# brown-palm/goal-force

Measured on AMD Instinct MI355X. Metric: frames_per_sec (81-frame video / (50-step denoise loop + VAE decode), Wan2.2-I2V-A14B 832x480x81f), higher is better.
Workload: dtype bf16

## Files before the change

goal_force_amd/csrc/gf_cross_fold.hip:

```cpp
#include "gf_common.h"

namespace {

constexpr int CF_HD = 128;
constexpr int CF_MAXK = 64;
constexpr int CF_THREADS = 256;
constexpr int CF_QB = 128;

__device__ __forceinline__ void cf_mfma32(f32x16& acc, const bf16x8& a, const bf16x8& b) {
    acc = __builtin_amdgcn_mfma_f32_32x32x16_bf16(a, b, acc, 0, 0, 0);
}

__global__ __launch_bounds__(CF_THREADS) void cross_probs_kernel(const u16* __restrict__ q, const u16* __restrict__ k, u16* __restrict__ pout,
                                                                 int q_len, int n_keys, int n_pad, int heads, long q_stride, long k_stride,
                                                                 long p_stride, float c, float last_key_bias) {
    __shared__ __attribute__((aligned(16))) char lds[CF_MAXK * 256];
    const int tid = threadIdx.x;
    const int lane = tid & 63, wave = tid >> 6;
    const int r = lane & 31, h = lane >> 5;
    const int head = blockIdx.y;
    const int q0 = blockIdx.x * CF_QB + wave * 32;
    const int halves = n_keys > 32 ? 2 : 1;

#pragma unroll
// ... 2 lines not shown
        const int row = idx >> 4, ch = idx & 15;
        u16x8 v8 = {0, 0, 0, 0, 0, 0, 0, 0};
        if (row < n_keys) v8 = *reinterpret_cast<const u16x8*>(k + (long)row * k_stride + head * CF_HD + ch * 8);
        const int sk = ((row & 3) << 2) | ((row >> 2) & 3);
        *(u16x8*)(lds + row * 256 + ((ch ^ sk) << 4)) = v8;
    }

    bf16x8 qf[8];
    {
        const int qr = min(q0 + r, q_len - 1);
        const u16* qp = q + (long)qr * q_stride + head * CF_HD + 8 * h;
#pragma unroll
        for (int kd = 0; kd < 8; ++kd) qf[kd] = *reinterpret_cast<const bf16x8*>(qp + 16 * kd);
    }
    __syncthreads();

    f32x16 sc[2];
#pragma unroll
    for (int e = 0; e < 16; ++e) {
        sc[0][e] = 0.f;
        sc[1][e] = 0.f;
    }
    const int sK = ((r & 3) << 2) | ((r >> 2) & 3);
#pragma unroll
    for (int kd = 0; kd < 8; ++kd) {
        const int off = 256 * r + 16 * ((2 * kd + h) ^ sK);
        cf_mfma32(sc[0], *(const bf16x8*)(lds + off), qf[kd]);
        if (halves == 2) cf_mfma32(sc[1], *(const bf16x8*)(lds + off + 32 * 256), qf[kd]);
    }

#pragma unroll
    for (int e = 0; e < 16; ++e) {
        const int key = 4 * h + (e & 3) + 8 * (e >> 2);
        if (key >= n_keys) sc[0][e] = -INFINITY;
        if (key + 32 >= n_keys) sc[1][e] = -INFINITY;
        if (key == n_keys - 1) sc[0][e] += last_key_bias;
        if (key + 32 == n_keys - 1) sc[1][e] += last_key_bias;
    }
    float mx = sc[0][0];
#pragma unroll
    for (int e = 1; e < 16; ++e) mx = fmaxf(mx, sc[0][e]);
#pragma unroll
    for (int e = 0; e < 16; ++e) mx = fmaxf(mx, sc[1][e]);
    mx = fmaxf(mx, __shfl_xor(mx, 32));
    const float mc = mx * c;
    float rs = 0.f;
#pragma unroll
    for (int e = 0; e < 16; ++e) {
        sc[0][e] = __builtin_amdgcn_exp2f(__builtin_fmaf(sc[0][e], c, -mc));
        sc[1][e] = __builtin_amdgcn_exp2f(__builtin_fmaf(sc[1][e], c, -mc));
        rs += sc[0][e] + sc[1][e];
    }
    const float l_tot = rs + __shfl_xor(rs, 32);
    const float inv = 1.0f / l_tot;
    float pl = 0.f;
#pragma unroll
    for (int e = 0; e < 16; ++e) {
        const int key = 4 * h + (e & 3) + 8 * (e >> 2);
        if (key == n_keys - 1) pl = sc[0][e];
        if (key + 32 == n_keys - 1) pl = sc[1][e];
    }
    pl += __shfl_xor(pl, 32);
    const float wl = pl * inv;
    const float wl_lo = wl - bf2f(f2bf(wl));

    const int qrow = q0 + r;
    if (qrow < q_len) {
        u16* prow = pout + (long)qrow * p_stride + (long)head * n_pad;
#pragma unroll
        for (int half = 0; half < 2; ++half)
#pragma unroll
            for (int g = 0; g < 4; ++g) {
                const int key = 32 * half + 8 * g + 4 * h;
                if (key < n_pad) {
                    float w4[4];
#pragma unroll
                    for (int i = 0; i < 4; ++i) w4[i] = key + i == n_keys ? wl_lo : sc[half][4 * g + i] * inv;
                    u32x2 pk;
                    pk[0] = pack2bf(w4[0], w4[1]);
                    pk[1] = pack2bf(w4[2], w4[3]);
                    *reinterpret_cast<u32x2*>(prow + key) = pk;
                }
            }
    }
}

constexpr int CFT_ROWS = 64;
__global__ __launch_bounds__(CF_THREADS) void cross_fold_table_kernel(const u16* __restrict__ v, const u16* __restrict__ w, u16* __restrict__ u,
                                                                      int n_keys, int n_pad, int n_out, long v_stride, long w_stride,
                                                                      long u_stride) {
    __shared__ __attribute__((aligned(16))) u16 vs[CF_MAXK * CF_HD];
    const int tid = threadIdx.x;
    const int head = blockIdx.y;
    for (int idx = tid; idx < n_pad * 16; idx += CF_THREADS) {
        const int row = idx >> 4, ch = idx & 15;
        u16x8 v8 = {0, 0, 0, 0, 0, 0, 0, 0};
        if (row <= n_keys) v8 = *reinterpret_cast<const u16x8*>(v + (long)min(row, n_keys - 1) * v_stride + head * CF_HD + ch * 8);
        *reinterpret_cast<u16x8*>(vs + row * CF_HD + ch * 8) = v8;
    }
    __syncthreads();
    const int n = blockIdx.x * CFT_ROWS + (tid >> 2), jg = tid & 3;
    if (n >= n_out) return;
    const int nj = n_pad >> 2;
    float acc[CF_MAXK / 4];
#pragma unroll
    for (int i = 0; i < CF_MAXK / 4; ++i) acc[i] = 0.f;
    const u16* wr = w + (long)n * w_stride + head * CF_HD;
    for (int d0 = 0; d0 < CF_HD; d0 += 8) {
        const u16x8 w8 = *reinterpret_cast<const u16x8*>(wr + d0);
        float wf[8];
#pragma unroll
        for (int e = 0; e < 8; ++e) wf[e] = bf2f(w8[e]);
#pragma unroll
        for (int i = 0; i < CF_MAXK / 4; ++i) {
            if (i < nj) {
                const u16x8 v8 = *reinterpret_cast<const u16x8*>(vs + (jg + 4 * i) * CF_HD + d0);
#pragma unroll
                for (int e = 0; e < 8; ++e) acc[i] = __builtin_fmaf(bf2f(v8[e]), wf[e], acc[i]);
            }
        }
    }
    u16* ur = u + (long)n * u_stride + (long)head * n_pad;
#pragma unroll
    for (int i = 0; i < CF_MAXK / 4; ++i) {
        const int j = jg + 4 * i;
        if (i < nj) ur[j] = j <= n_keys ? f2bf(acc[i]) : (u16)0;
    }
}

}

extern "C" GF_API int gf_cross_probs(const void* q, const void* k, void* p, int64_t q_len, int64_t n_keys, int64_t n_pad, int64_t heads,
                                     int64_t head_dim, int64_t q_stride, int64_t k_stride, int64_t p_stride, float scale,
                                     float last_key_multiplicity, void* stream) {
    GF_CHECK_ARG(q && k && p, "gf_cross_probs: null pointer");
    if (head_dim != CF_HD) {
        gf_set_error("gf_cross_probs: head_dim=%ld unsupported (kernel is built for 128)", (long)head_dim);
        return GF_ERR_UNSUPPORTED;
    }
    GF_CHECK_ARG(q_len >= 0 && q_len < (1 << 30) && heads > 0 && heads < 65536, "gf_cross_probs: bad sizes q=%ld heads=%ld", (long)q_len,
                 (long)heads);
    GF_CHECK_ARG(n_keys >= 1 && n_pad % 16 == 0 && n_pad > n_keys && n_pad <= CF_MAXK,
                 "gf_cross_probs: 1 <= n_keys=%ld < n_pad=%ld <= 64, n_pad a multiple of 16", (long)n_keys, (long)n_pad);
    GF_CHECK_ARG(q_stride % 8 == 0 && k_stride % 8 == 0 && p_stride % 4 == 0 && q_stride >= heads * CF_HD && k_stride >= heads * CF_HD &&
                     p_stride >= heads * n_pad,
                 "gf_cross_probs: strides must cover the rows (q, k: multiples of 8; p: of 4, >= heads * n_pad)");
    GF_CHECK_ARG(gf_aligned16(q) && gf_aligned16(k) && ((uintptr_t)p & 7u) == 0, "gf_cross_probs: alignment (q, k 16 bytes, p 8 bytes)");
    GF_CHECK_ARG(scale > 0.f && last_key_multiplicity >= 1.0f, "gf_cross_probs: scale > 0, multiplicity >= 1");
    if (q_len == 0) return GF_OK;
    const float c = scale * 1.4426950408889634f;
    const float bias = last_key_multiplicity != 1.0f ? log2f(last_key_multiplicity) / c : 0.f;
    const dim3 grid((unsigned)((q_len + CF_QB - 1) / CF_QB), (unsigned)heads);
    hipLaunchKernelGGL(cross_probs_kernel, grid, dim3(CF_THREADS), 0, (hipStream_t)stream, (const u16*)q, (const u16*)k, (u16*)p,
                       (int)q_len, (int)n_keys, (int)n_pad, (int)heads, (long)q_stride, (long)k_stride, (long)p_stride, c, bias);
    GF_CHECK_LAUNCH("gf_cross_probs");
    return GF_OK;
}

extern "C" GF_API int gf_cross_fold_table(const void* v, const void* w_o, void* u, int64_t n_keys, int64_t n_pad, int64_t heads,
                                          int64_t head_dim, int64_t n_out, int64_t v_stride, int64_t w_stride, int64_t u_stride,
                                          void* stream) {
    GF_CHECK_ARG(v && w_o && u, "gf_cross_fold_table: null pointer");
    if (head_dim != CF_HD) {
        gf_set_error("gf_cross_fold_table: head_dim=%ld unsupported (kernel is built for 128)", (long)head_dim);
        return GF_ERR_UNSUPPORTED;
    }
    GF_CHECK_ARG(heads > 0 && heads < 65536 && n_out > 0 && n_out < (1 << 30), "gf_cross_fold_table: bad sizes heads=%ld N=%ld", (long)heads,
                 (long)n_out);
    GF_CHECK_ARG(n_keys >= 1 && n_pad % 16 == 0 && n_pad > n_keys && n_pad <= CF_MAXK,
                 "gf_cross_fold_table: 1 <= n_keys=%ld < n_pad=%ld <= 64, n_pad a multiple of 16", (long)n_keys, (long)n_pad);
    GF_CHECK_ARG(v_stride % 8 == 0 && w_stride % 8 == 0 && v_stride >= heads * CF_HD && w_stride >= heads * CF_HD && u_stride >= heads * n_pad,
                 "gf_cross_fold_table: strides must cover the rows (v, w_o: multiples of 8; u >= heads * n_pad)");
    GF_CHECK_ARG(gf_aligned16(v) && gf_aligned16(w_o) && ((uintptr_t)u & 1u) == 0, "gf_cross_fold_table: alignment");
    const dim3 grid((unsigned)((n_out + CFT_ROWS - 1) / CFT_ROWS), (unsigned)heads);
    hipLaunchKernelGGL(cross_fold_table_kernel, grid, dim3(CF_THREADS), 0, (hipStream_t)stream, (const u16*)v, (const u16*)w_o, (u16*)u,
                       (int)n_keys, (int)n_pad, (int)n_out, (long)v_stride, (long)w_stride, (long)u_stride);
    GF_CHECK_LAUNCH("gf_cross_fold_table");
    return GF_OK;
}
```

goal_force_amd/dit.py:

```python
from __future__ import annotations

import math
from typing import Optional, Tuple

import torch
import torch.nn as nn

from . import ops
from ._lib import GoalForceError


def precompute_freqs_cis(dim: int, end: int = 1024, theta: float = 10000.0):
    freqs = 1.0 / (theta ** (torch.arange(0, dim, 2)[: (dim // 2)].double() / dim))
    freqs = torch.outer(torch.arange(end), freqs)
    return torch.polar(torch.ones_like(freqs), freqs)


def precompute_freqs_cis_3d(dim: int, end: int = 1024, theta: float = 10000.0):
    return (precompute_freqs_cis(dim - 2 * (dim // 3), end, theta),
            precompute_freqs_cis(dim // 3, end, theta),
            precompute_freqs_cis(dim // 3, end, theta))


class RopeTable:
# ... 260 lines not shown
            q = linear(xin, self.q)
            ops.rmsnorm_rope(q, self.norm_q.weight, q_cos, q_sin, self.head_dim, self.norm_q.eps)
            hq = sp.heads_start(q, self.num_heads)
            return sp.attention_started(hq, hk, hv, self.num_heads, tuple(q.shape), scale=attn_scale, backend="sage" if sage else "flash")
        q, k = linear(xin, self.q), linear(xin, self.k)
        if keep is not None and keep.get("wide"):
            keep["qp"], keep["kp"] = q, k
            q, k = q.clone(), k.clone()
        ops.rmsnorm_rope(q, self.norm_q.weight, q_cos, q_sin, self.head_dim, self.norm_q.eps)
        ops.rmsnorm_rope(k, self.norm_k.weight, rope.cos, rope.sin, self.head_dim, self.norm_k.eps)
        if sp is None and keep is None and not fp8 and x2.is_cuda and self.v.weight.shape[0] >= 512 \
                and ops.vt32_ok(x2.shape[0], self.num_heads, self.head_dim):
            return attn(q, k, None, self.num_heads, vt=ops.linear_vt32(x2, self.v.weight, self.v.bias), scale=attn_scale)
        if sp is None and keep is None and fp8 and xin.is_cuda and self.v.weight.shape[0] >= 512 and self.v.weight.shape[1] % 128 == 0 \
                and ops.vt32_ok(xin.shape[0], self.num_heads, self.head_dim):
            if self.v._gf_w8_key != param_key(self.v.weight):
                self.v._gf_w8 = ops.cast_fp8(self.v.weight.detach().contiguous())
                self.v._gf_w8_key = param_key(self.v.weight)
            return attn(q, k, None, self.num_heads, vt=ops.linear_vt32_fp8(xin.x8, xin.scale, self.v._gf_w8, self.v.bias), scale=attn_scale)
        v = linear(xin, self.v)
        if sp is not None:
            return sp.attention(q, k, v, self.num_heads, scale=attn_scale, backend="sage" if sage else "flash")
        if keep is not None:
            keep["attn"], keep["lse"] = ops.flash_attn_lse(q, k, v, self.num_heads, scale=attn_scale)
            if keep.get("wide"):
                keep["v"] = v
            return keep["attn"]
        return attn(q, k, v, self.num_heads, scale=attn_scale)

    def forward(self, x, freqs):
        x2 = _tokens2d(x)
        a = self.attend(x2, _as_rope(freqs, x.device))
        return linear(a, self.o).view(x.shape)


class CrossAttention(nn.Module):

    def __init__(self, dim: int, num_heads: int, eps: float = 1e-6, has_image_input: bool = False):
        super().__init__()
        if has_image_input:
            raise NotImplementedError("has_image_input=True (CLIP image tokens) is outside the Goal-Force path")
        self.dim, self.num_heads, self.head_dim = dim, num_heads, dim // num_heads
        self.q, self.k, self.v, self.o = (nn.Linear(dim, dim) for _ in range(4))
        self.norm_q, self.norm_k = RMSNorm(dim, eps=eps), RMSNorm(dim, eps=eps)
        self.has_image_input = False

    def context_kv(self, ctx2: torch.Tensor, fold: bool = True, pad_n: Optional[int] = None):
        m = 1
        if fold and ctx2.is_cuda and ops._OPT["fold_pad_keys"]:
            n = pad_run(ctx2) if pad_n is None else pad_n
            if ctx2.shape[0] - n >= 2 and n + 1 < ops.VT_MIN_KV:
                m = ctx2.shape[0] - n
                ctx2 = ctx2[: n + 1]
        cin = QuantizedInput(ctx2) if getattr(self.k, "_gf_w8", None) is not None else ctx2
        k, v = linear(cin, self.k), linear(cin, self.v)
        ops.rmsnorm_rope(k, self.norm_k.weight, None, None, self.head_dim, self.norm_k.eps)
        return k, v, m

    def attend(self, x2, kv):
        q = linear(x2, self.q)
        ops.rmsnorm_rope(q, self.norm_q.weight, None, None, self.head_dim, self.norm_q.eps)
        return ops.flash_attn(q, kv[0], kv[1], self.num_heads, last_key_mult=kv[2] if len(kv) > 2 else 1)

    FOLD_K_MAX = 2560

    def fold_ok(self, kv) -> bool:
        if not ops._OPT["fold_cross_o"] or torch.is_grad_enabled() or len(kv) < 3 or kv[2] == 1 or self.head_dim != 128:
            return False
        if getattr(self.o, "_gf_w8", None) is not None:
            return False
        n = kv[0].shape[0]
        k = self.num_heads * self.fold_pad(n)
        return n <= ops.CROSS_FOLD_MAX_KEYS and k <= self.FOLD_K_MAX and k % 64 == 0

    @staticmethod
    def fold_pad(n_keys: int) -> int:
        return -(-(n_keys + 1) // 16) * 16

    def fold_table(self, kv):
        return ops.cross_fold_table(kv[1], self.o.weight, self.num_heads, self.fold_pad(kv[0].shape[0]))

    def attend_probs(self, x2, kv):
        q = linear(x2, self.q)
        ops.rmsnorm_rope(q, self.norm_q.weight, None, None, self.head_dim, self.norm_q.eps)
        return ops.cross_probs(q, kv[0], self.num_heads, self.fold_pad(kv[0].shape[0]), last_key_mult=kv[2])

    def forward(self, x: torch.Tensor, y: torch.Tensor):
        x2 = _tokens2d(x)
        a = self.attend(x2, self.context_kv(_tokens2d(y)))
        return linear(a, self.o).view(x.shape)


class GateModule(nn.Module):

    def forward(self, x, gate, residual):
        if x.shape != residual.shape:
            raise GoalForceError("GateModule: x and residual must have the same shape")
        d = x.shape[-1]
        g = gate.reshape(-1, d)
        if x.dim() == 3 and g.shape[0] == x.shape[0] and x.shape[0] > 1:
            return torch.stack([ops.gate_residual(x[b], g[b].contiguous(), residual[b]) for b in range(x.shape[0])])
        if g.shape[0] != 1:
            raise GoalForceError("GateModule: gate must be [B or 1, 1, D] (per-token gates are outside the Goal-Force path)")
        return ops.gate_residual(x, g[0].contiguous(), residual)


class DiTBlock(nn.Module):

    def __init__(self, has_image_input: bool, dim: int, num_heads: int, ffn_dim: int, eps: float = 1e-6):
        super().__init__()
        self.dim, self.num_heads, self.ffn_dim, self.eps = dim, num_heads, ffn_dim, eps
        self.self_attn = SelfAttention(dim, num_heads, eps)
        self.cross_attn = CrossAttention(dim, num_heads, eps, has_image_input=has_image_input)
        self.norm1 = nn.LayerNorm(dim, eps=eps, elementwise_affine=False)
        self.norm2 = nn.LayerNorm(dim, eps=eps, elementwise_affine=False)
        self.norm3 = nn.LayerNorm(dim, eps=eps)
        self.ffn = nn.Sequential(nn.Linear(dim, ffn_dim), nn.GELU(approximate="tanh"), nn.Linear(ffn_dim, dim))
        self.modulation = nn.Parameter(torch.randn(1, 6, dim) / dim ** 0.5)
        self.gate = GateModule()

    def forward(self, x, context, t_mod, freqs, context_kv=None, out=None, sp=None, keep=None, self_attn_memo=None,
                fold_pad_keys=True, pad_n=None, dense_attn=False):
        if t_mod.dim() == 4:
            raise NotImplementedError("per-token t_mod (seperated_timestep) is outside the Goal-Force path")
        x2 = _tokens2d(x)
        rope = _as_rope(freqs, x.device)
        mod = ops.modulation(self.modulation, t_mod.contiguous(), onep_mask=0b010010)
        fp8 = getattr(self.ffn[0], "_gf_w8", None) is not None
        if self_attn_memo is not None and "x" in self_attn_memo:
            x_new = self_attn_memo.pop("x")
            ev = self_attn_memo.pop("ev", None)
            if ev is not None:
                torch.cuda.current_stream(x_new.device).wait_event(ev)
                x_new.record_stream(torch.cuda.current_stream(x_new.device))
            if out is not None:
                x_new = out.copy_(x_new)
            h = None if fp8 else torch.empty_like(x2)
        else:
            if fp8:
                h = QuantizedInput.layernorm(x2, scale1p=mod[1], shift=mod[0], eps=self.eps)
            else:
                h = ops.layernorm_modulate(x2, scale1p=mod[1], shift=mod[0], eps=self.eps)
            a = self.self_attn.attend(h, rope, sp, keep, dense=dense_attn)
            x_new = out if out is not None else torch.empty_like(x2)
            linear(a, self.self_attn.o, epilogue=ops.EPI_BIAS_GATE_RESID, resid=x2, gate=mod[2], out=x_new)
            if keep is not None and keep.get("wide"):
                keep["x1"] = x_new.clone()
            if self_attn_memo is not None:
                self_attn_memo["x"] = x_new.clone()
                if x_new.is_cuda:
                    self_attn_memo["ev"] = torch.cuda.Event()
                    self_attn_memo["ev"].record(torch.cuda.current_stream(x_new.device))
        if fp8:
            h = QuantizedInput.layernorm(x_new, weight=self.norm3.weight, bias=self.norm3.bias, eps=self.eps)
        else:
            ops.layernorm_modulate(x_new, weight=self.norm3.weight, bias=self.norm3.bias, eps=self.eps, out=h)
        if context_kv is None:
            context_kv = self.cross_attn.context_kv(_tokens2d(context), fold=fold_pad_keys and keep is None, pad_n=pad_n)
        ca = self.cross_attn
        if keep is None and not fp8 and ca.fold_ok(context_kv):
            u = context_kv[3] if len(context_kv) > 3 else ca.fold_table(context_kv)
            ops.gemm(ca.attend_probs(h, context_kv), u, ca.o.bias, epilogue=ops.EPI_BIAS_RESID, resid=x_new, out=x_new)
        else:
            a = ca.attend(h, context_kv)
            linear(a, ca.o, epilogue=ops.EPI_BIAS_RESID, resid=x_new, out=x_new)
        if keep is not None and keep.get("wide"):
# ... 133 lines not shown
```

goal_force_amd/ops.py:

```python
from __future__ import annotations

import math

import torch

from . import _lib
from ._lib import (EPI_BIAS, EPI_BIAS_GATE_RESID, EPI_BIAS_GELU_TANH, EPI_BIAS_MUL, EPI_BIAS_RESID, EPI_BIAS_SILU,
                   GoalForceError)

__all__ = [
    "modulation", "layernorm_modulate", "rmsnorm_rope", "gate_residual", "gemm", "flash_attn", "flash_attn_sparse", "BlockMap", "block_means", "block_means_coherence", "block_map_scores", "block_map_select", "block_map_from_qk", "patchify_im2col", "unpatchify",
    "cfg_euler_step", "act", "add", "sub", "rel_l1", "force_map",
    "EPI_BIAS", "EPI_BIAS_GELU_TANH", "EPI_BIAS_GATE_RESID", "EPI_BIAS_RESID", "EPI_BIAS_SILU", "EPI_BIAS_MUL",
]

_BF16 = torch.bfloat16
_FP8 = torch.float8_e4m3fn

PROFILE_ATTN = None
PROFILE_GEMM = None
PROFILE_CONV = None


def _stream(t: torch.Tensor):
# ... 140 lines not shown
    xv, rows, dim, xs = _rows2d(x, "rmsnorm_rope.x")
    if cos is not None:
        _req(cos, "rmsnorm_rope.cos", torch.float32)
        _req(sin, "rmsnorm_rope.sin", torch.float32)
        if cos.shape != (rows, head_dim // 2) or sin.shape != cos.shape or not cos.is_contiguous() \
                or not sin.is_contiguous():
            raise GoalForceError(f"rmsnorm_rope: cos/sin must be contiguous [{rows}, {head_dim // 2}]")
    _lib.check(_lib.load().gf_rmsnorm_rope(_ptr(xv), _ptr(weight), _ptr(cos), _ptr(sin), rows, dim, head_dim, xs,
                                           float(eps), _stream(x)), "gf_rmsnorm_rope")
    return x


def modulate(x, shift, scale):
    _req(x, "modulate.x")
    xv, rows, dim, xs = _rows2d(x, "modulate.x")
    _vec(shift, "modulate.shift", dim, required=True)
    _vec(scale, "modulate.scale", dim, required=True)
    out = torch.empty(x.shape, dtype=_BF16, device=x.device)
    ov, _, _, os_ = _rows2d(out, "modulate.out")
    _lib.check(_lib.load().gf_modulate(_ptr(xv), _ptr(ov), _ptr(scale), _ptr(shift), rows, dim, xs, os_, _stream(x)), "gf_modulate")
    return out


def gate_residual(x, gate, residual):
    _req(x, "gate_residual.x")
    _req(residual, "gate_residual.residual")
    xv, rows, dim, xs = _rows2d(x, "gate_residual.x")
    rv, rrows, rdim, rs = _rows2d(residual, "gate_residual.residual")
    if (rrows, rdim) != (rows, dim):
        raise GoalForceError(f"gate_residual: residual must match x [{rows}, {dim}]")
    _vec(gate, "gate_residual.gate", dim, required=True)
    out = torch.empty(x.shape, dtype=_BF16, device=x.device)
    ov, _, _, os_ = _rows2d(out, "gate_residual.out")
    _lib.check(_lib.load().gf_gate_residual(_ptr(xv), _ptr(gate), _ptr(rv), _ptr(ov), rows, dim, xs, rs, os_, _stream(x)),
               "gf_gate_residual")
    return out


def rope_apply(x, cos, sin, head_dim):
    _req(x, "rope_apply.x")
    xv, rows, dim, xs = _rows2d(x, "rope_apply.x")
    for n, t in (("cos", cos), ("sin", sin)):
        _req(t, f"rope_apply.{n}", torch.float32)
        if tuple(t.shape) != (rows, head_dim // 2) or not t.is_contiguous():
            raise GoalForceError(f"rope_apply.{n}: expected contiguous [{rows}, {head_dim // 2}] fp32")
    out = torch.empty(x.shape, dtype=_BF16, device=x.device)
    ov, _, _, os_ = _rows2d(out, "rope_apply.out")
    _lib.check(_lib.load().gf_rope_apply(_ptr(xv), _ptr(ov), _ptr(cos), _ptr(sin), rows, dim, head_dim, xs, os_, _stream(x)),
               "gf_rope_apply")
    return out


def _gemm(a, w, row_scale, bias, epilogue, resid, gate, out):
    av, M, K, lda, N, ldw = _linear_operands(a, w, row_scale)
    if out is None:
        out = torch.empty(a.shape[:-1] + (N,), dtype=_BF16, device=a.device)
    ov, Mo, No, ldc = _rows2d(out, "gemm[_fp8].out")
    if (Mo, No) != (M, N):
        raise GoalForceError(f"gemm[_fp8].out: expected [{M}, {N}], got [{Mo}, {No}]")
    ldr = 0
    if resid is not None:
        _req(resid, "gemm[_fp8].resid")
        resid, Mr, Nr, ldr = _rows2d(resid, "gemm[_fp8].resid")
        if (Mr, Nr) != (M, N):
            raise GoalForceError(f"gemm[_fp8].resid: expected [{M}, {N}], got [{Mr}, {Nr}]")
    _vec(gate, "gemm[_fp8].gate", N)
    _vec(bias, "gemm[_fp8].bias", N)
    lib = _lib.load()
    fn, scale = (lib.gf_gemm_bf16, ()) if row_scale is None else (lib.gf_gemm_fp8, (_ptr(row_scale),))
    with _timed(PROFILE_GEMM, M, N, K, int(epilogue)):
        _lib.check(fn(_ptr(av), lda, _ptr(w), ldw, *scale, _ptr(bias), _ptr(ov), ldc, M, N, K, int(epilogue), _ptr(resid), ldr,
                      _ptr(gate), _stream(a)), fn.__name__)
    return out


def gemm(a, w, bias=None, epilogue=EPI_BIAS, resid=None, gate=None, out=None):
    return _gemm(a, w, None, bias, epilogue, resid, gate, out)


VT_MIN_KV = 2048
_LIB_DEFAULTS = {"prefer_8wave": 0, "a4_stagger": 2, "a4_group_m": 0, "conv_nb": 0, "conv_gather": 0, "conv_direct": 1, "vae_rms3": 1,
                 "attn_fixed_max": 1}
_OPT = {"attn_k3": True, "vt_from_gemm": True, "conv_padded": True, "fold_pad_keys": True, "attn_q_prescale": True, "vae_attn_offset": True,
        "fold_cross_o": True}


def lib_option(name: str) -> int:
    import ctypes
    v = ctypes.c_int(0)
    _lib.check(_lib.load().gf_get_option(name.encode(), ctypes.byref(v)), f"gf_get_option({name})")
    return int(v.value)


class options:

    def __init__(self, **kv):
        for k in kv:
            if k not in _OPT and k not in _LIB_DEFAULTS:
                raise GoalForceError(f"ops.options: unknown option {k!r}")
        self.kv, self.old = kv, {}

    @staticmethod
    def _apply_one(k, v):
        if k in _OPT:
            _OPT[k] = bool(v)
        else:
            _lib.check(_lib.load().gf_set_option(k.encode(), int(v)), f"gf_set_option({k})")

    def __enter__(self):
        self.old = {}
        try:
            for k, v in self.kv.items():
                old = _OPT[k] if k in _OPT else lib_option(k)
                self._apply_one(k, v)
                self.old[k] = old
        except BaseException:
            self.__exit__(None, None, None)
            raise
        return self

    def __exit__(self, *exc):
        for k, v in reversed(list(self.old.items())):
            self._apply_one(k, v)
        self.old = {}
        return False


_VT_WS = {}


def _vt_workspace(numel, device):
    key = (device.index, torch.cuda.current_stream(device).cuda_stream)
    ws = _VT_WS.get(key)
    if ws is None or ws.numel() < numel:
        ws = _VT_WS[key] = torch.empty((numel,), dtype=_BF16, device=device)
    return ws


def _vt_shape(skv, num_heads, head_dim):
    return skv >= VT_MIN_KV and head_dim == 128 and num_heads * 128 * kv_pad(skv) < 2 ** 31


def vt32_ok(skv, num_heads, head_dim):
    return _vt_shape(skv, num_heads, head_dim) and _OPT["attn_k3"] and _OPT["vt_from_gemm"]


def _linear_vt32(x, w, x_scale, bias):
    xv, skv, K, ldx, N, ldw = _linear_operands(x, w, x_scale)
    _vec(bias, "linear_vt32[_fp8].bias", N)
    vt = _vt_workspace(N * kv_pad(skv), x.device)
    lib = _lib.load()
    fn, scale = (lib.gf_linear_vt32, ()) if x_scale is None else (lib.gf_linear_vt32_fp8, (_ptr(x_scale),))
    _lib.check(fn(_ptr(xv), ldx, *scale, _ptr(w), ldw, _ptr(bias), _ptr(vt), skv, kv_pad(skv), N, K, _stream(x)), fn.__name__)
    return vt


def linear_vt32(x, weight, bias):
    return _linear_vt32(x, weight, None, bias)


def linear_vt32_fp8(x8, x_scale, w8, bias):
    if x_scale is None:
        raise GoalForceError("linear_vt32_fp8.x_scale: required")
    return _linear_vt32(x8, w8, x_scale, bias)


last_attn_flags = None
# ... 453 lines not shown
    k8 = torch.empty((kv_pad8, num_heads * 128), dtype=torch.int8, device=k.device)
    sc = torch.empty((num_heads, kv_pad8 // SAGE_KBLK), dtype=torch.float32, device=k.device)
    _lib.check(_lib.load().gf_sage_quant_k(_ptr(k), ldk, _ptr(mu), _ptr(k8), _ptr(sc), skv, num_heads, _stream(k)), "gf_sage_quant_k")
    return k8, sc, mu


def sage_quant_vt(v, num_heads, vt=None, kv_len=None):
    if vt is None:
        skv, ldv = _sage_rows(v, "sage_quant_vt.v", num_heads)
        src, vt_in = v, 0
    else:
        _req(vt, "sage_quant_vt.vt")
        if kv_len is None or kv_len < 1:
            raise GoalForceError("sage_quant_vt: a V^T input needs kv_len")
        skv, ldv, src, vt_in = kv_len, kv_pad(kv_len), vt, 1
        if vt.numel() < num_heads * 128 * ldv:
            raise GoalForceError("sage_quant_vt.vt: buffer smaller than heads*128*kv_pad")
    kv_pad8 = -(-skv // SAGE_T) * SAGE_T
    vt8 = torch.empty((num_heads * 128, kv_pad8), dtype=torch.uint8, device=src.device)
    sc = torch.empty((num_heads, 128), dtype=torch.float32, device=src.device)
    _lib.check(_lib.load().gf_sage_quant_vt(_ptr(src), ldv, vt_in, _ptr(vt8), _ptr(sc), _ptr(_sage_scratch(num_heads, src.device)), skv,
                                            num_heads, _stream(src)), "gf_sage_quant_vt")
    return vt8, sc


def sage_attn_quantized(q8, q_scale, k8, k_scale, vt8, v_scale, kv_len, num_heads, scale=None, out=None):
    sq = q8.shape[0]
    scale = _sage_scale(scale)
    if out is None:
        out = torch.empty((sq, num_heads * 128), dtype=_BF16, device=q8.device)
    _lib.check(_lib.load().gf_sage_attn_fwd(_ptr(q8), _ptr(q_scale), _ptr(k8), _ptr(k_scale), _ptr(vt8), _ptr(v_scale), _ptr(out),
                                            out.stride(0), sq, kv_len, num_heads, scale, _stream(q8)), "gf_sage_attn_fwd")
    return out


def sage_attn(q, k, v, num_heads, scale=None, vt=None, out=None):
    scale = _sage_scale(scale)
    sq, ldq = _sage_rows(q, "sage_attn.q", num_heads)
    skv, ldk = _sage_rows(k, "sage_attn.k", num_heads)
    if vt is None:
        sv, ldv = _sage_rows(v, "sage_attn.v", num_heads)
        if sv != skv:
            raise GoalForceError(f"sage_attn: k has {skv} keys, v {sv}")
        src, vt_in = v, 0
    else:
        _req(vt, "sage_attn.vt")
        ldv, src, vt_in = kv_pad(skv), vt, 1
        if vt.numel() < num_heads * 128 * ldv:
            raise GoalForceError("sage_attn.vt: buffer smaller than heads*128*kv_pad")
    out = _out(out, "sage_attn.out", sq, num_heads * 128, q.device)
    if out.stride(0) % 8:
        raise GoalForceError("sage_attn.out: row stride must be a multiple of 8 elements")
    lib = _lib.load()
    nbytes = int(lib.gf_sage_workspace_bytes(sq, skv, num_heads))
    key = (q.device.index, torch.cuda.current_stream(q.device).cuda_stream)
    ws = _SAGE_WS.get(key)
    if ws is None or ws.numel() < nbytes:
        ws = _SAGE_WS[key] = torch.empty((nbytes,), dtype=torch.uint8, device=q.device)
    with _timed(PROFILE_ATTN, sq, skv, num_heads):
        _lib.check(lib.gf_sage_attn(_ptr(q), ldq, _ptr(k), ldk, _ptr(src), ldv, vt_in, _ptr(out), out.stride(0), sq, skv, num_heads,
                                    scale, _ptr(ws), _stream(q)), "gf_sage_attn")
    return out


CROSS_FOLD_MAX_KEYS = 63


def cross_probs(q, k, num_heads, n_pad, last_key_mult=1, scale=None, out=None):
    _mat(q, "cross_probs.q")
    _mat(k, "cross_probs.k")
    sq, hd_all = q.shape
    n_keys = k.shape[0]
    head_dim = hd_all // num_heads
    if k.shape[1] != hd_all or head_dim * num_heads != hd_all:
        raise GoalForceError("cross_probs: q/k shape mismatch")
    out = _out(out, "cross_probs.out", sq, num_heads * n_pad, q.device)
    if scale is None:
        scale = 1.0 / math.sqrt(head_dim)
    _lib.check(_lib.load().gf_cross_probs(_ptr(q), _ptr(k), _ptr(out), sq, n_keys, n_pad, num_heads, head_dim, q.stride(0), k.stride(0),
                                          out.stride(0), float(scale), float(last_key_mult), _stream(q)), "gf_cross_probs")
    return out


def cross_fold_table(v, w_o, num_heads, n_pad):
    _mat(v, "cross_fold_table.v")
    n_keys, hd_all = v.shape
    N, ldw = _weight(w_o, "cross_fold_table.w_o", hd_all)
    if hd_all % num_heads:
        raise GoalForceError(f"cross_fold_table: {hd_all} columns do not divide into {num_heads} heads")
    u = torch.empty((N, num_heads * n_pad), dtype=_BF16, device=v.device)
    _lib.check(_lib.load().gf_cross_fold_table(_ptr(v), _ptr(w_o), _ptr(u), n_keys, n_pad, num_heads, hd_all // num_heads, N, v.stride(0),
                                               ldw, u.stride(0), _stream(v)), "gf_cross_fold_table")
    return u


def flash_attn_lse(q, k, v, num_heads, scale=None):
    for n, t in (("q", q), ("k", k), ("v", v)):
        _mat(t, f"flash_attn_lse.{n}")
    sq, hd_all = q.shape
    skv = k.shape[0]
    head_dim = hd_all // num_heads
    if k.shape[1] != hd_all or v.shape != k.shape or head_dim * num_heads != hd_all:
        raise GoalForceError("flash_attn_lse: q/k/v shape mismatch")
    if scale is None:
        scale = 1.0 / math.sqrt(head_dim)
    out = torch.empty((sq, hd_all), dtype=_BF16, device=q.device)
    lse = torch.empty((sq, num_heads), dtype=torch.float32, device=q.device)
    lib = _lib.load()
    if _vt_shape(skv, num_heads, head_dim):
        _vt_attn(lib, q, k, v, None, out, lse, sq, skv, num_heads, head_dim, scale, _OPT["attn_k3"])
        return out, lse
    _lib.check(lib.gf_flash_attn_fwd_lse(_ptr(q), _ptr(k), _ptr(v), _ptr(out), _ptr(lse), sq, skv, num_heads, head_dim,
                                         q.stride(0), k.stride(0), v.stride(0), out.stride(0), float(scale),
                                         _stream(q)), "gf_flash_attn_fwd_lse")
    return out, lse


def flash_attn_bwd(q, k, v, o, dout, lse, num_heads, scale=None, need_dkv=True):
    for n, t in (("q", q), ("k", k), ("v", v), ("o", o), ("dout", dout)):
        _mat(t, f"flash_attn_bwd.{n}")
    sq, hd_all = q.shape
    skv = k.shape[0]
    head_dim = hd_all // num_heads
    if scale is None:
        scale = 1.0 / math.sqrt(head_dim)
    if lse.dtype != torch.float32 or tuple(lse.shape) != (sq, num_heads) or not lse.is_contiguous():
        raise GoalForceError("flash_attn_bwd.lse: expected contiguous fp32 [Sq, heads]")
    dq = torch.empty_like(q, memory_format=torch.contiguous_format)
    dk = torch.empty((skv, hd_all), dtype=_BF16, device=q.device) if need_dkv else None
    dv = torch.empty((skv, hd_all), dtype=_BF16, device=q.device) if need_dkv else None
    lib = _lib.load()
    ws = torch.empty((int(lib.gf_flash_attn_bwd_workspace_bytes(sq, skv, num_heads)),), dtype=torch.uint8, device=q.device)
    _lib.check(lib.gf_flash_attn_bwd(_ptr(q), _ptr(k), _ptr(v), _ptr(o), _ptr(dout), _ptr(lse), _ptr(ws), _ptr(dq),
                                             _ptr(dk) if need_dkv else None, _ptr(dv) if need_dkv else None, sq, skv, num_heads, head_dim,
                                             q.stride(0), k.stride(0), v.stride(0), o.stride(0), dout.stride(0), dq.stride(0),
                                             dk.stride(0) if need_dkv else hd_all, dv.stride(0) if need_dkv else hd_all, float(scale),
                                             _stream(q)), "gf_flash_attn_bwd")
    return dq, dk, dv


def patchify_im2col(src0, src1=None, kpad=None):
    _req(src0, "patchify.src0")
    if src0.dim() != 4 or not src0.is_contiguous():
        raise GoalForceError("patchify.src0: expected contiguous [c,F,H,W]")
    c0, F, H, W = src0.shape
    c1 = 0
    if src1 is not None:
        _req(src1, "patchify.src1")
        if src1.dim() != 4 or not src1.is_contiguous() or src1.shape[1:] != src0.shape[1:]:
            raise GoalForceError("patchify.src1: expected contiguous [c1,F,H,W] matching src0")
        c1 = src1.shape[0]
    if kpad is None:
        kpad = -(-((c0 + c1) * 4) // 64) * 64
    out = torch.empty((F * (H // 2) * (W // 2), kpad), dtype=_BF16, device=src0.device)
    _lib.check(_lib.load().gf_patchify_im2col(_ptr(src0), c0, _ptr(src1), c1, _ptr(out), F, H, W, kpad,
                                              _stream(src0)), "gf_patchify_im2col")
    return out


def unpatchify(tokens, c, f, h, w):
    _req(tokens, "unpatchify.tokens")
    if tokens.shape != (f * h * w, 4 * c) or not tokens.is_contiguous():
        raise GoalForceError(f"unpatchify.tokens: expected contiguous [{f * h * w}, {4 * c}]")
    out = torch.empty((c, f, 2 * h, 2 * w), dtype=_BF16, device=tokens.device)
    _lib.check(_lib.load().gf_unpatchify(_ptr(tokens), _ptr(out), c, f, h, w, _stream(tokens)), "gf_unpatchify")
    return out
# ... 445 lines not shown
```

include/goalforce.h:

```cpp
#ifndef GOALFORCE_H
#define GOALFORCE_H

#include <stdint.h>

#if defined(GF_BUILD)
#define GF_API __attribute__((visibility("default")))
#else
#define GF_API
#endif

#ifdef __cplusplus
extern "C" {
#endif

typedef enum {
    GF_OK = 0,
    GF_ERR_INVALID_ARG = -1,
    GF_ERR_UNSUPPORTED = -2,
    GF_ERR_LAUNCH = -3
} gf_status;

GF_API const char* gf_version(void);
GF_API const char* gf_last_error(void);
#define GF_ABI_VERSION 20
GF_API int gf_abi_version(void);
GF_API int gf_set_option(const char* name, int value);
GF_API int gf_get_option(const char* name, int* value);
GF_API void gf_reset_options(void);

GF_API int gf_layernorm_modulate(const void* x, void* out, const void* weight, const void* bias,
                          const void* scale1p, const void* shift,
                          int64_t rows, int64_t dim, int64_t x_stride, int64_t out_stride,
                          float eps, void* stream);

GF_API int gf_modulation(const void* param, const void* t, void* out, int64_t k, int64_t dim,
                         int64_t t_rows, uint32_t onep_mask, void* stream);

GF_API int gf_rmsnorm_rope(void* x, const void* weight, const float* cos_tab, const float* sin_tab,
                    int64_t rows, int64_t dim, int64_t head_dim, int64_t x_stride,
                    float eps, void* stream);

typedef enum {
    GF_EPI_BIAS = 0,
    GF_EPI_BIAS_GELU_TANH = 1,
    GF_EPI_BIAS_GATE_RESID = 2,
    GF_EPI_BIAS_RESID = 3,
    GF_EPI_BIAS_SILU = 4,
    GF_EPI_BIAS_MUL = 5
} gf_epilogue;

GF_API int gf_gemm_bf16(const void* A, int64_t lda, const void* W, int64_t ldw, const void* bias,
                 void* C, int64_t ldc, int64_t M, int64_t N, int64_t K,
                 int epilogue, const void* resid, int64_t ldr, const void* gate,
                 void* stream);

GF_API int gf_gemm_bf16_batched(const void* A, int64_t lda, int64_t strideA, const void* W, int64_t ldw, int64_t strideW, void* C,
                                int64_t ldc, int64_t strideC, int64_t M, int64_t N, int64_t K, int64_t batch, void* stream);

GF_API int gf_flash_attn_fwd(const void* q, const void* k, const void* v, void* o,
                      int64_t q_len, int64_t kv_len, int64_t heads, int64_t head_dim,
                      int64_t q_stride, int64_t k_stride, int64_t v_stride, int64_t o_stride,
                      float scale, void* stream);

GF_API int gf_transpose_v(const void* v, int64_t v_stride, void* vt, int64_t kv_len, int64_t kv_pad, int64_t heads, void* stream);
GF_API int gf_flash_attn_fwd_vt(const void* q, const void* k, const void* vt, void* o, float* lse,
                         int64_t q_len, int64_t kv_len, int64_t kv_pad, int64_t heads, int64_t head_dim,
                         int64_t q_stride, int64_t k_stride, int64_t o_stride, float scale, void* stream);

GF_API int gf_transpose_v32(const void* v, int64_t v_stride, void* vt, int64_t kv_len, int64_t kv_pad, int64_t heads, void* stream);
GF_API int gf_flash_attn_fwd_vt32(const void* q, const void* k, const void* vt, void* o, float* lse,
                                  int64_t q_len, int64_t kv_len, int64_t kv_pad, int64_t heads, int64_t head_dim,
                                  int64_t q_stride, int64_t k_stride, int64_t o_stride, float scale, void* stream);

GF_API int gf_flash_attn_fwd_vt32_sparse(const void* q, const void* k, const void* vt, void* o, float* lse,
                                         const int32_t* row_ptr, const int32_t* tile_idx, const int32_t* head_map, int64_t n_maps,
                                         int64_t q_len, int64_t kv_len, int64_t kv_pad, int64_t heads, int64_t head_dim,
                                         int64_t q_stride, int64_t k_stride, int64_t o_stride, float scale, void* stream);

GF_API int gf_flash_attn_fwd_vt32_fm(const void* q, const void* k, const void* vt, void* o, float* lse, int32_t* flags,
                                     int64_t q_len, int64_t kv_len, int64_t kv_pad, int64_t heads, int64_t head_dim,
                                     int64_t q_stride, int64_t k_stride, int64_t o_stride, float scale, void* stream);
GF_API int gf_flash_attn_fwd_vt32_sparse_fm(const void* q, const void* k, const void* vt, void* o, float* lse, int32_t* flags,
                                            const int32_t* row_ptr, const int32_t* tile_idx, const int32_t* head_map, int64_t n_maps,
                                            int64_t q_len, int64_t kv_len, int64_t kv_pad, int64_t heads, int64_t head_dim,
                                            int64_t q_stride, int64_t k_stride, int64_t o_stride, float scale, void* stream);

GF_API int gf_linear_vt32(const void* x, int64_t ldx, const void* w, int64_t ldw, const void* bias, void* vt,
                          int64_t kv_len, int64_t kv_pad, int64_t N, int64_t K, void* stream);

GF_API int gf_flash_attn_fwd_lastmult(const void* q, const void* k, const void* v, void* o, int64_t q_len, int64_t kv_len,
                                      int64_t heads, int64_t head_dim, int64_t q_stride, int64_t k_stride, int64_t v_stride,
                                      int64_t o_stride, float scale, float last_key_multiplicity, void* stream);

GF_API int gf_cross_probs(const void* q, const void* k, void* p, int64_t q_len, int64_t n_keys, int64_t n_pad, int64_t heads,
                          int64_t head_dim, int64_t q_stride, int64_t k_stride, int64_t p_stride, float scale,
                          float last_key_multiplicity, void* stream);

GF_API int gf_cross_fold_table(const void* v, const void* w_o, void* u, int64_t n_keys, int64_t n_pad, int64_t heads, int64_t head_dim,
                               int64_t n_out, int64_t v_stride, int64_t w_stride, int64_t u_stride, void* stream);

GF_API int gf_flash_attn_fwd_lse(const void* q, const void* k, const void* v, void* o, float* lse,
                          int64_t q_len, int64_t kv_len, int64_t heads, int64_t head_dim,
                          int64_t q_stride, int64_t k_stride, int64_t v_stride, int64_t o_stride,
                          float scale, void* stream);
GF_API int64_t gf_flash_attn_bwd_workspace_bytes(int64_t q_len, int64_t kv_len, int64_t heads);
GF_API int gf_flash_attn_bwd(const void* q, const void* k, const void* v, const void* o, const void* dout,
                      const float* lse, void* workspace, void* dq, void* dk, void* dv,
                      int64_t q_len, int64_t kv_len, int64_t heads, int64_t head_dim,
                      int64_t q_stride, int64_t k_stride, int64_t v_stride, int64_t o_stride, int64_t do_stride,
                      int64_t dq_stride, int64_t dk_stride, int64_t dv_stride, float scale, void* stream);

GF_API int gf_layernorm_bwd(const void* x, int64_t x_stride, const void* dy, int64_t dy_stride, const void* g, void* dx,
                            int64_t dx_stride, float* dg_acc, float* db_acc, int64_t rows, int64_t dim, float eps, void* stream);
GF_API int gf_rmsnorm_rope_bwd(const void* x, int64_t x_stride, const void* dy, int64_t dy_stride, const void* weight,
                               const float* cos_tab, const float* sin_tab, void* dx, int64_t dx_stride, float* dw_acc,
                               int64_t rows, int64_t dim, int64_t head_dim, float eps, void* stream);
GF_API int gf_colsum(const void* a, int64_t lda, const void* b, int64_t ldb, const void* gate, void* out, int64_t ldo,
                     float* acc, int64_t rows, int64_t cols, void* stream);
GF_API int gf_act_bwd(const void* u, const void* df, void* du, int64_t n, int kind, void* stream);
GF_API int gf_mse_loss(const void* pred, const void* target, void* dpred, float* loss, int64_t n, float weight, void* stream);
GF_API int gf_adamw_step(void* param, const void* grad, float* exp_avg, float* exp_avg_sq, int64_t n, float lr, float beta1,
                         float beta2, float eps, float weight_decay, int64_t step, float grad_scale, void* stream);
GF_API int gf_f32_to_bf16(const float* src, void* dst, int64_t n, void* stream);
GF_API int gf_sumsq(const void* x, int64_t n, float* acc, void* stream);

GF_API int64_t gf_block_map_workspace_bytes(int64_t q_len, int64_t kv_len, int64_t heads);
GF_API int64_t gf_block_map_select_workspace_bytes(int64_t n_qblocks, int64_t n_tiles, int64_t heads);
GF_API int gf_block_means(const void* x, int64_t ldx, float* mean, int64_t rows, int64_t heads, int64_t block, void* stream);
GF_API int gf_block_map_scores(const float* q_mean, const float* k_mean, float* scores, int64_t q_len, int64_t kv_len, int64_t heads,
                               float scale, void* stream);
GF_API int gf_block_map_select(const float* scores, const uint32_t* forced, int32_t* row_ptr, int32_t* tile_idx, int32_t* head_map,
                               float* kept, void* ws, int64_t n_qblocks, int64_t n_tiles, int64_t heads, float mass, void* stream);
GF_API int gf_block_map_from_qk(const void* q, int64_t ldq, const void* k, int64_t ldk, const uint32_t* forced, int32_t* row_ptr,
                                int32_t* tile_idx, int32_t* head_map, float* scores, float* kept, void* ws, int64_t q_len,
                                int64_t kv_len, int64_t heads, float scale, float mass, void* stream);
GF_API int64_t gf_block_map_gated_workspace_bytes(int64_t q_len, int64_t kv_len, int64_t heads);
GF_API int gf_block_means_coh(const void* x, int64_t ldx, float* mean, float* coh, int64_t rows, int64_t heads, int64_t block,
                              void* stream);
GF_API int gf_block_map_select_gated(const float* scores, const uint32_t* forced, const float* q_coh, const float* k_coh,
                                     int32_t* row_ptr, int32_t* tile_idx, int32_t* head_map, float* kept, void* ws, int64_t n_qblocks,
                                     int64_t n_tiles, int64_t heads, float mass, float q_min, float k_min, void* stream);
GF_API int gf_block_map_from_qk_gated(const void* q, int64_t ldq, const void* k, int64_t ldk, const uint32_t* forced, int32_t* row_ptr,
                                      int32_t* tile_idx, int32_t* head_map, float* scores, float* kept, float* q_coh_out,
                                      float* k_coh_out, void* ws, int64_t q_len, int64_t kv_len, int64_t heads, float scale, float mass,
                                      float q_min, float k_min, void* stream);

GF_API int gf_patchify_im2col(const void* src0, int64_t c0, const void* src1, int64_t c1,
                       void* out, int64_t F, int64_t H, int64_t W, int64_t kpad, void* stream);

GF_API int gf_unpatchify(const void* tokens, void* out, int64_t c, int64_t f, int64_t h, int64_t w,
                  void* stream);

GF_API int gf_cfg_euler_step(void* latents, const void* posi, const void* nega,
                      float cfg_scale, float dsigma, int64_t n, void* stream);

GF_API int gf_act(const void* x, void* out, int64_t n, int kind, void* stream);

GF_API int gf_add_bf16(const void* a, const void* b, void* out, int64_t n, void* stream);

GF_API int gf_sub_bf16(const void* a, const void* b, void* out, int64_t n, void* stream);
GF_API int gf_rel_l1_bf16(const void* cur, const void* prev, int64_t n, void* sums, void* stream);

GF_API int gf_force_map(void* out, int64_t frames, int64_t H, int64_t W,
                 const int32_t* channels, const float* params, const float* centers,
                 int64_t n_blobs, int clamp01, void* stream);


GF_API int gf_vae_prep_latent(const void* z, int64_t sc, int64_t st, int64_t sy, int64_t sx,
                              const void* mean, const void* inv_std, void* out,
                              int64_t C, int64_t T, int64_t H, int64_t W, int64_t cpad, void* stream);

GF_API int gf_vae_im2col(const void* src, const void* cache, void* out, int64_t T_out, int64_t H, int64_t W,
                         int64_t C, int64_t kt, int64_t ks, int mode, int64_t t_stride, int64_t t_off,
                         int64_t kpad, void* stream);

GF_API int gf_conv3d_bf16(const void* src, const void* cache, const void* Wm, int64_t ldw, const void* bias,
                          void* out, int64_t ldc, int64_t T_in, int64_t T_out, int64_t H, int64_t W, int64_t C,
                          int kt, int ks, int mode, int t_stride, int t_off, int64_t N, int64_t K, int epilogue,
                          const void* resid, int64_t ldr, void* stream);
// ... 83 lines not shown
```

Before: 0.6343.

## Fuse cross-attention query RMSNorm into row-wise cross probabilities kernel

```diff
diff --git a/goal_force_amd/csrc/gf_cross_fold.hip b/goal_force_amd/csrc/gf_cross_fold.hip
--- a/goal_force_amd/csrc/gf_cross_fold.hip
+++ b/goal_force_amd/csrc/gf_cross_fold.hip
@@ -108,6 +108,152 @@
                     *reinterpret_cast<u32x2*>(prow + key) = pk;
                 }
             }
+    }
+}
+
+constexpr int CR_ROWS = 16;
+#ifndef GF_CROSS_ROWS_WAVES
+#define GF_CROSS_ROWS_WAVES 8
+#endif
+constexpr int CR_WAVES = GF_CROSS_ROWS_WAVES;
+constexpr int CR_MAX_HPW = 40 / CR_WAVES;
+
+template <int HPW, int NT>
+__global__ __launch_bounds__(64 * CR_WAVES) void cross_probs_rows_kernel(const u16* __restrict__ q, const u16* __restrict__ norm_w,
+                                                                         const u16* __restrict__ k, u16* __restrict__ pout, int q_len,
+                                                                         int n_keys, int n_pad, long q_stride, long k_stride,
+                                                                         long p_stride, float inv_dim, float eps, float c,
+                                                                         float last_key_bias) {
+    constexpr int HEADS = HPW * CR_WAVES;
+    __shared__ __attribute__((aligned(16))) float ws[HEADS * CF_HD];
+    __shared__ float part[CR_WAVES][CR_ROWS];
+    const int tid = threadIdx.x;
+    const int lane = tid & 63, wave = tid >> 6;
+    const int n = lane & 15, g = lane >> 4;
+    const int qrow = blockIdx.x * CR_ROWS + n;
+    const bool live = qrow < q_len;
+
+    u32x4 qf[HPW][4];
+    {
+        const u16* qp = q + (long)min(qrow, q_len - 1) * q_stride + wave * HPW * CF_HD + 8 * g;
+#pragma unroll
+        for (int hh = 0; hh < HPW; ++hh)
+#pragma unroll
+            for (int kd = 0; kd < 4; ++kd) qf[hh][kd] = *reinterpret_cast<const u32x4*>(qp + hh * CF_HD + 32 * kd);
+    }
+    const u16* kbase[NT];
+#pragma unroll
+    for (int t = 0; t < NT; ++t) kbase[t] = k + (long)min(16 * t + n, n_keys - 1) * k_stride + wave * HPW * CF_HD + 8 * g;
+    u16x8 a8[NT][4];
+#pragma unroll
+    for (int t = 0; t < NT; ++t)
+#pragma unroll
+        for (int kd = 0; kd < 4; ++kd) a8[t][kd] = *reinterpret_cast<const u16x8*>(kbase[t] + 32 * kd);
+    for (int i = tid; i < HEADS * (CF_HD / 8); i += 64 * CR_WAVES) {
+        const u16x8 w8 = *reinterpret_cast<const u16x8*>(norm_w + 8 * i);
+        *reinterpret_cast<f32x4*>(ws + 8 * i) = f32x4{bf2f(w8[0]), bf2f(w8[1]), bf2f(w8[2]), bf2f(w8[3])};
+        *reinterpret_cast<f32x4*>(ws + 8 * i + 4) = f32x4{bf2f(w8[4]), bf2f(w8[5]), bf2f(w8[6]), bf2f(w8[7])};
+    }
+
+    float s = 0.f;
+#pragma unroll
+    for (int hh = 0; hh < HPW; ++hh)
+#pragma unroll
+        for (int kd = 0; kd < 4; ++kd)
+#pragma unroll
+            for (int j = 0; j < 4; ++j) {
+                const float f0 = __uint_as_float(qf[hh][kd][j] << 16), f1 = __uint_as_float(qf[hh][kd][j] & 0xffff0000u);
+                s = __builtin_fmaf(f0, f0, s);
+                s = __builtin_fmaf(f1, f1, s);
+            }
+    s += __shfl_xor(s, 16);
+    s += __shfl_xor(s, 32);
+    if (g == 0) part[wave][n] = s;
+    __syncthreads();
+    float tot = part[0][n];
+#pragma unroll
+    for (int w = 1; w < CR_WAVES; ++w) tot += part[w][n];
+    const float rstd = 1.0f / sqrtf(tot * inv_dim + eps);
+
+    const u16x8 zero8 = {0, 0, 0, 0, 0, 0, 0, 0};
+    u16* prow = pout + (long)qrow * p_stride;
+#pragma unroll
+    for (int hh = 0; hh < HPW; ++hh) {
+        const int head = wave * HPW + hh;
+        bf16x8 qn[4];
+#pragma unroll
+        for (int kd = 0; kd < 4; ++kd) {
+            const float* wp = ws + head * CF_HD + 32 * kd + 8 * g;
+            const f32x4 wa = *reinterpret_cast<const f32x4*>(wp), wb = *reinterpret_cast<const f32x4*>(wp + 4);
+            const float wf[8] = {wa[0], wa[1], wa[2], wa[3], wb[0], wb[1], wb[2], wb[3]};
+            u32x4 o;
+#pragma unroll
+            for (int j = 0; j < 4; ++j) {
+                const unsigned x2 = qf[hh][kd][j];
+                const unsigned n2 = pack2bf(__uint_as_float(x2 << 16) * rstd, __uint_as_float(x2 & 0xffff0000u) * rstd);
+                o[j] = pack2bf(__uint_as_float(n2 << 16) * wf[2 * j], __uint_as_float(n2 & 0xffff0000u) * wf[2 * j + 1]);
+            }
+            qn[kd] = __builtin_bit_cast(bf16x8, o);
+        }
+        f32x4 sc[NT];
+#pragma unroll
+        for (int t = 0; t < NT; ++t) {
+            sc[t] = f32x4{0.f, 0.f, 0.f, 0.f};
+            const bool in = 16 * t + n < n_keys;
+#pragma unroll
+            for (int kd = 0; kd < 4; ++kd)
+                sc[t] = __builtin_amdgcn_mfma_f32_16x16x32_bf16(__builtin_bit_cast(bf16x8, in ? a8[t][kd] : zero8), qn[kd], sc[t], 0, 0, 0);
+        }
+        if (hh + 1 < HPW) {
+#pragma unroll
+            for (int t = 0; t < NT; ++t)
+#pragma unroll
+                for (int kd = 0; kd < 4; ++kd) a8[t][kd] = *reinterpret_cast<const u16x8*>(kbase[t] + (hh + 1) * CF_HD + 32 * kd);
+        }
+
+        float mx = -INFINITY;
+#pragma unroll
+        for (int t = 0; t < NT; ++t)
+#pragma unroll
+            for (int i = 0; i < 4; ++i) {
+                const int key = 16 * t + 4 * g + i;
+                if (key >= n_keys) sc[t][i] = -INFINITY;
+                if (key == n_keys - 1) sc[t][i] += last_key_bias;
+                mx = fmaxf(mx, sc[t][i]);
+            }
+        mx = fmaxf(mx, __shfl_xor(mx, 16));
+        mx = fmaxf(mx, __shfl_xor(mx, 32));
+        const float mc = mx * c;
+        float rs = 0.f, pl = 0.f;
+#pragma unroll
+        for (int t = 0; t < NT; ++t)
+#pragma unroll
+            for (int i = 0; i < 4; ++i) {
+                sc[t][i] = __builtin_amdgcn_exp2f(__builtin_fmaf(sc[t][i], c, -mc));
+                rs += sc[t][i];
+                if (16 * t + 4 * g + i == n_keys - 1) pl = sc[t][i];
+            }
+        rs += __shfl_xor(rs, 16);
+        rs += __shfl_xor(rs, 32);
+        const float inv = 1.0f / rs;
+        pl += __shfl_xor(pl, 16);
+        pl += __shfl_xor(pl, 32);
+        const float wl = pl * inv;
+        const float wl_lo = wl - bf2f(f2bf(wl));
+
+        if (live) {
+#pragma unroll
+            for (int t = 0; t < NT; ++t) {
+                const int key = 16 * t + 4 * g;
+                float w4[4];
+#pragma unroll
+                for (int i = 0; i < 4; ++i) w4[i] = key + i == n_keys ? wl_lo : sc[t][i] * inv;
+                u32x2 pk;
+                pk[0] = pack2bf(w4[0], w4[1]);
+                pk[1] = pack2bf(w4[2], w4[3]);
+                *reinterpret_cast<u32x2*>(prow + (long)head * n_pad + key) = pk;
+            }
+        }
     }
 }
 
@@ -183,6 +329,54 @@
     return GF_OK;
 }
 
+extern "C" GF_API int gf_cross_probs_rows(const void* q, const void* norm_w, float eps, const void* k, void* p, int64_t q_len, int64_t n_keys,
+                                          int64_t n_pad, int64_t heads, int64_t head_dim, int64_t q_stride, int64_t k_stride,
+                                          int64_t p_stride, float scale, float last_key_multiplicity, void* stream) {
+    GF_CHECK_ARG(q && norm_w && k && p, "gf_cross_probs_rows: null pointer");
+    if (head_dim != CF_HD) {
+        gf_set_error("gf_cross_probs_rows: head_dim=%ld unsupported (kernel is built for 128)", (long)head_dim);
+        return GF_ERR_UNSUPPORTED;
+    }
+    GF_CHECK_ARG(q_len >= 0 && q_len < (1 << 30) && heads > 0 && heads < 65536, "gf_cross_probs_rows: bad sizes q=%ld heads=%ld", (long)q_len,
+                 (long)heads);
+    if (heads % CR_WAVES != 0 || heads / CR_WAVES > CR_MAX_HPW) {
+        gf_set_error("gf_cross_probs_rows: heads=%ld unsupported (a multiple of %d, at most %d)", (long)heads, CR_WAVES, CR_WAVES * CR_MAX_HPW);
+        return GF_ERR_UNSUPPORTED;
+    }
+    GF_CHECK_ARG(n_keys >= 1 && n_pad % 16 == 0 && n_pad > n_keys && n_pad <= CF_MAXK,
+                 "gf_cross_probs_rows: 1 <= n_keys=%ld < n_pad=%ld <= 64, n_pad a multiple of 16", (long)n_keys, (long)n_pad);
+    GF_CHECK_ARG(q_stride % 8 == 0 && k_stride % 8 == 0 && p_stride % 4 == 0 && q_stride >= heads * CF_HD && k_stride >= heads * CF_HD &&
+                     p_stride >= heads * n_pad,
+                 "gf_cross_probs_rows: strides must cover the rows (q, k: multiples of 8; p: of 4, >= heads * n_pad)");
+    GF_CHECK_ARG(gf_aligned16(q) && gf_aligned16(k) && gf_aligned16(norm_w) && ((uintptr_t)p & 7u) == 0,
+                 "gf_cross_probs_rows: alignment (q, k, norm_w 16 bytes, p 8 bytes)");
+    GF_CHECK_ARG(scale > 0.f && last_key_multiplicity >= 1.0f && eps >= 0.f, "gf_cross_probs_rows: scale > 0, multiplicity >= 1, eps >= 0");
+    if (q_len == 0) return GF_OK;
+    const float c = scale * 1.4426950408889634f;
+    const float bias = last_key_multiplicity != 1.0f ? log2f(last_key_multiplicity) / c : 0.f;
+    const float inv_dim = 1.0f / (float)(heads * CF_HD);
+    const dim3 grid((unsigned)((q_len + CR_ROWS - 1) / CR_ROWS));
+#define GF_CR_CASE(HPW)                                                                                                              \
+    case HPW:                                                                                                                        \
+        GF_CR_TILES(HPW, 1) GF_CR_TILES(HPW, 2) GF_CR_TILES(HPW, 3) GF_CR_TILES(HPW, 4)                                               \
+        break;
+#define GF_CR_TILES(HPW, NT)                                                                                                         \
+    if (n_pad == 16 * NT)                                                                                                            \
+        hipLaunchKernelGGL((cross_probs_rows_kernel<HPW, NT>), grid, dim3(64 * CR_WAVES), 0, (hipStream_t)stream, (const u16*)q,            \
+                           (const u16*)norm_w, (const u16*)k, (u16*)p, (int)q_len, (int)n_keys, (int)n_pad, (long)q_stride,          \
+                           (long)k_stride, (long)p_stride, inv_dim, eps, c, bias);
+    switch ((int)(heads / CR_WAVES)) {
+        GF_CR_CASE(1) GF_CR_CASE(2) GF_CR_CASE(3) GF_CR_CASE(4) GF_CR_CASE(5)
+#if GF_CROSS_ROWS_WAVES == 4
+        GF_CR_CASE(6) GF_CR_CASE(7) GF_CR_CASE(8) GF_CR_CASE(9) GF_CR_CASE(10)
+#endif
+    }
+#undef GF_CR_CASE
+#undef GF_CR_TILES
+    GF_CHECK_LAUNCH("gf_cross_probs_rows");
+    return GF_OK;
+}
+
 extern "C" GF_API int gf_cross_fold_table(const void* v, const void* w_o, void* u, int64_t n_keys, int64_t n_pad, int64_t heads,
                                           int64_t head_dim, int64_t n_out, int64_t v_stride, int64_t w_stride, int64_t u_stride,
                                           void* stream) {
diff --git a/goal_force_amd/dit.py b/goal_force_amd/dit.py
--- a/goal_force_amd/dit.py
+++ b/goal_force_amd/dit.py
@@ -366,6 +366,9 @@
 
     def attend_probs(self, x2, kv):
         q = linear(x2, self.q)
+        if ops._OPT["fuse_cross_qnorm"] and ops.cross_probs_rows_ok(self.num_heads, self.head_dim):
+            return ops.cross_probs_rows(q, self.norm_q.weight, kv[0], self.num_heads, self.fold_pad(kv[0].shape[0]), last_key_mult=kv[2],
+                                        eps=self.norm_q.eps)
         ops.rmsnorm_rope(q, self.norm_q.weight, None, None, self.head_dim, self.norm_q.eps)
         return ops.cross_probs(q, kv[0], self.num_heads, self.fold_pad(kv[0].shape[0]), last_key_mult=kv[2])
 
diff --git a/goal_force_amd/ops.py b/goal_force_amd/ops.py
--- a/goal_force_amd/ops.py
+++ b/goal_force_amd/ops.py
@@ -246,7 +246,7 @@
 _LIB_DEFAULTS = {"prefer_8wave": 0, "a4_stagger": 2, "a4_group_m": 0, "conv_nb": 0, "conv_gather": 0, "conv_direct": 1, "vae_rms3": 1,
                  "attn_fixed_max": 1}
 _OPT = {"attn_k3": True, "vt_from_gemm": True, "conv_padded": True, "fold_pad_keys": True, "attn_q_prescale": True, "vae_attn_offset": True,
-        "fold_cross_o": True}
+        "fold_cross_o": True, "fuse_cross_qnorm": True}
 
 
 def lib_option(name: str) -> int:
@@ -866,6 +866,31 @@
     return out
 
 
+CROSS_ROWS_HEAD_STEP, CROSS_ROWS_MAX_HEADS = 8, 40
+
+
+def cross_probs_rows_ok(num_heads, head_dim) -> bool:
+    return head_dim == 128 and num_heads % CROSS_ROWS_HEAD_STEP == 0 and 0 < num_heads <= CROSS_ROWS_MAX_HEADS
+
+
+def cross_probs_rows(q, norm_weight, k, num_heads, n_pad, last_key_mult=1, eps=1e-6, scale=None, out=None):
+    _mat(q, "cross_probs_rows.q")
+    _mat(k, "cross_probs_rows.k")
+    sq, hd_all = q.shape
+    n_keys = k.shape[0]
+    head_dim = hd_all // num_heads
+    if k.shape[1] != hd_all or head_dim * num_heads != hd_all:
+        raise GoalForceError("cross_probs_rows: q/k shape mismatch")
+    _vec(norm_weight, "cross_probs_rows.norm_weight", hd_all, required=True)
+    out = _out(out, "cross_probs_rows.out", sq, num_heads * n_pad, q.device)
+    if scale is None:
+        scale = 1.0 / math.sqrt(head_dim)
+    _lib.check(_lib.load().gf_cross_probs_rows(_ptr(q), _ptr(norm_weight), float(eps), _ptr(k), _ptr(out), sq, n_keys, n_pad, num_heads,
+                                               head_dim, q.stride(0), k.stride(0), out.stride(0), float(scale), float(last_key_mult),
+                                               _stream(q)), "gf_cross_probs_rows")
+    return out
+
+
 def cross_fold_table(v, w_o, num_heads, n_pad):
     _mat(v, "cross_fold_table.v")
     n_keys, hd_all = v.shape
diff --git a/include/goalforce.h b/include/goalforce.h
--- a/include/goalforce.h
+++ b/include/goalforce.h
@@ -95,6 +95,10 @@
 GF_API int gf_cross_probs(const void* q, const void* k, void* p, int64_t q_len, int64_t n_keys, int64_t n_pad, int64_t heads,
                           int64_t head_dim, int64_t q_stride, int64_t k_stride, int64_t p_stride, float scale,
                           float last_key_multiplicity, void* stream);
+
+GF_API int gf_cross_probs_rows(const void* q, const void* norm_w, float eps, const void* k, void* p, int64_t q_len, int64_t n_keys,
+                               int64_t n_pad, int64_t heads, int64_t head_dim, int64_t q_stride, int64_t k_stride, int64_t p_stride,
+                               float scale, float last_key_multiplicity, void* stream);
 
 GF_API int gf_cross_fold_table(const void* v, const void* w_o, void* u, int64_t n_keys, int64_t n_pad, int64_t heads, int64_t head_dim,
                                int64_t n_out, int64_t v_stride, int64_t w_stride, int64_t u_stride, void* stream);
```

After: 0.6332. About the same (-0.2%).
